# HyeonwooNoh/VQA-Transfer-ExternalData

Hardware: AMD Instinct MI355X
Metric: VQA train samples/sec (img+question) at bs512 (higher is better)
Workload: dtype f32

## Files before the change

vqa-transfer-externaldata_amd/csrc/fusion_model.hip:

```cpp
#include <stdlib.h>
#include <string.h>

#include <string>
#include <vector>

#include "gemm_args.h"
#include "gru_encoder.h"
#include "keep_launch.h"

namespace {

inline bool has_tuned_head(int mt) { return mt == VQA_MODEL_VQA_ALL2 || mt == VQA_MODEL_VQA_ALL; }
inline bool train_loss_masked(int mt) { return mt != VQA_MODEL_STANDARD; }
inline bool bf16_routed(int mt) { return mt == VQA_MODEL_VLMAP_ANSWER || mt == VQA_MODEL_STANDARD; }
inline bool feat16(const vqa_dims_t& d) { return (d.flags & VQA_FLAG_BF16_FEATURES) != 0; }

void legacy_vqa_layout(Layout& L, const vqa_dims_t& d, int64_t& gw);

Layout make_layout(const vqa_dims_t& d) {
    Layout L;
    const int64_t B = d.B, R = d.R, D = d.D, H = d.H, T = d.T, W = d.W, A = d.A;
    L.add("V_ft", B * R * D, feat16(d) ? 2 : 4);
    L.add("num_V_ft", B);
    L.add("pre_v", B * R * H);
// ... 244 lines not shown
int run_chains(const Ctx& c, int64_t B, Fn fn) {
    Chains& ch = gru_chains();
    int n = ch.n;
    while (n > 1 && B < 64 * (int64_t)n) --n;
    if (n <= 1) return fn(0, (int64_t)0, B, c.st);
    if (hipEventRecord(ch.fork, c.st) != hipSuccess) return VQA_ERR_LAUNCH;
    int rc = VQA_OK, launched = 0;
    for (int i = 1; i < n && rc == VQA_OK; ++i) {
        int64_t lo, hi;
        chain_rows(B, n, i, &lo, &hi);
        if (hipStreamWaitEvent(ch.s[i], ch.fork, 0) != hipSuccess) { rc = VQA_ERR_LAUNCH; break; }
        launched = i;
        if (ch.delay_us > 0.f) rc = vqa_stream_delay_us(ch.delay_us * (float)i, ch.s[i]);
        if (rc == VQA_OK) rc = fn(i, lo, hi - lo, ch.s[i]);
    }
    if (rc == VQA_OK) {
        int64_t lo, hi;
        chain_rows(B, n, 0, &lo, &hi);
        rc = fn(0, lo, hi - lo, c.st);
    }
    for (int i = 1; i <= launched; ++i)
        if (hipEventRecord(ch.join[i], ch.s[i]) != hipSuccess || hipStreamWaitEvent(c.st, ch.join[i], 0) != hipSuccess)
            rc = rc == VQA_OK ? VQA_ERR_LAUNCH : rc;
    return rc;
}
bool fork_side(const Ctx& c, Side& sd) {
    if (!sd.ok) return false;
    return hipEventRecord(sd.fork, c.st) == hipSuccess && hipStreamWaitEvent(sd.s, sd.fork, 0) == hipSuccess;
}
bool join_side_record(Side& sd) { return hipEventRecord(sd.join, sd.s) == hipSuccess; }


int gemm_f32(const Ctx& c, int tA, int tB, int64_t M, int64_t N, int64_t K, const float* A, int lda, const float* B,
             int ldb, float* C, int ldc, const float* bias = nullptr, const float* D = nullptr, int ldd = 0) {
    return vqa_gemm_f32_ex(tA, tB, (int)M, (int)N, (int)K, A, lda, B, ldb, C, ldc, bias, D, ldd, 0, c.gemm_ws(),
                           c.gemm_ws_floats(), c.lane ? side_max_blocks() : 0, c.st);
}
int gemm(const Ctx& c, int tA, int tB, int64_t M, int64_t N, int64_t K, const float* A, int lda, const float* B,
         int ldb, float* C, int ldc, const float* bias = nullptr, const float* D = nullptr, int ldd = 0) {
    if (c.d.flags & VQA_FLAG_BF16_GEMM)
        return vqa_gemm_bf16(tA, tB, (int)M, (int)N, (int)K, A, lda, B, ldb, C, ldc, bias, D, ldd, 0, c.gemm_ws(),
                             c.gemm_ws_floats(), c.lane ? side_max_blocks() : 0, c.st);
    return gemm_f32(c, tA, tB, M, N, K, A, lda, B, ldb, C, ldc, bias, D, ldd);
}
int gemm_x(const Ctx& c, int tA, int64_t M, int64_t N, int64_t K, const float* x, int ldx, const float* B, int ldb, float* C,
           int ldc, const float* bias = nullptr) {
    if (feat16(c.d) && x == c.f("V_ft"))
        return vqa_gemm_bf16_a16(tA, 0, (int)M, (int)N, (int)K, c.u16("V_ft"), ldx, B, ldb, C, ldc, bias, nullptr, 0, 0,
                                 c.gemm_ws(), c.gemm_ws_floats(), c.lane ? side_max_blocks() : 0, c.st);
    return gemm(c, tA, 0, M, N, K, x, ldx, B, ldb, C, ldc, bias);
}
int colsum(const Ctx& c, const float* X, int64_t M, int64_t N, int ldx, float* out) {
    return vqa_colsum(X, (int)M, (int)N, ldx, out, c.colsum_ws(), c.colsum_ws_floats(), c.st);
}
auto f32(const Ctx& c) { return [&c](auto... a) { return gemm_f32(c, a...); }; }
GruCell fw_cell(const vqa_params_t* p) { return {p->gru_wg, p->gru_bg, p->gru_wc, p->gru_bc}; }
GruCell bw_cell(const vqa_params_t* p) { return {p->gru_bw_wg, p->gru_bw_bg, p->gru_bw_wc, p->gru_bw_bc}; }

bool dims_ok(const vqa_dims_t* d) {
    if (!(d && d->B > 0 && d->R > 0 && d->D > 0 && d->H > 0 && d->T > 0 && d->W > 0 && d->A > 0 && d->Vq > 0 &&
          d->N_img > 0 && d->model_type >= VQA_MODEL_VLMAP_ANSWER && d->model_type <= VQA_MODEL_LEGACY_VQA))
        return false;
    if ((d->flags & VQA_FLAG_BF16_GEMM) && (!bf16_routed(d->model_type) || (d->flags & VQA_FLAG_FUSED_GATHER))) return false;
    if ((d->flags & VQA_FLAG_BF16_FEATURES) && !(d->flags & VQA_FLAG_BF16_GEMM)) return false;
    if (d->flags & VQA_PT_FLAG_BF16_ENCODER) return false;
    if (d->model_type == VQA_MODEL_LEGACY_VQA)
        return d->map_dim > 0 && d->La > 0 && d->H % 4 == 0 && d->D % 4 == 0 && d->map_dim % 4 == 0 && d->W % 4 == 0 && d->H <= 1024 && d->Vq > 3;
    if (d->model_type == VQA_MODEL_BI) return d->H % 8 == 0;
    if (d->model_type == VQA_MODEL_ENT)
        return d->num_marginal > 0 && d->ent_cols > 0 && d->ent_cols <= d->A && d->ent_cols <= 4096 &&
               (int64_t)d->B * d->num_marginal * (2 * (int64_t)d->H > d->ent_cols ? 2 * (int64_t)d->H : d->ent_cols) < (1ll << 30);
    return true;
}
inline int64_t pooled_dim(const vqa_dims_t& d) { return d.model_type == VQA_MODEL_ADAPT ? d.H : d.D; }

struct KeepSite {
    const uint8_t* mask;
    bool seeded;
    uint64_t seed, off;
    KeepSrc src(float keep_prob, int64_t row_len) const {
        return seeded ? KeepSrc::seeded(seed, off, row_len, keep_prob) : KeepSrc::bytes(mask, keep_prob);
    }
};
const KeepSite NO_KEEP = {nullptr, false, 0, 0};

KeepSite keep_site(const vqa_batch_t* bt, int site) {
    const bool sd = (bt->keep_seeded & site) != 0;
    switch (site) {
// ... 202 lines not shown
    return VQA_OK;
}

extern "C" int vqa_vtail_set_mode(int mode) {
    g_vtail_mode = mode < 0 ? -1 : (mode ? 1 : 0);
    return vtail_mode();
}

extern "C" int vqa_gru_h0skip_set_mode(int mode) {
    g_h0skip_mode = mode < 0 ? -1 : (mode & 3);
    return h0skip_mode();
}

namespace {

struct Step {
    const vqa_dims_t& d;
    const vqa_params_t* const P;
    const vqa_params_t* const G;
    const vqa_batch_t* const bt;
    const Layout L;
    const Ctx c;
    const int mt;
    const int64_t B, R, D, H, T, W, A;
    const int64_t Dp;
    GruTape enc[2];
    Side* sd = nullptr;
    bool forked = false;
    bool fuse_gather = false, visual_late = false;
    const float* q_ft = nullptr;
    const float* qv_in = nullptr;
    const float* lin_in = nullptr;
    bool pair = false;

    Step(const vqa_dims_t* dims, const vqa_params_t* P_, const vqa_params_t* G_, const vqa_batch_t* bt_, void* workspace,
         void* stream)
        : d(*dims), P(P_), G(G_), bt(bt_), L(make_layout(*dims)),
          c{{L, static_cast<char*>(workspace)}, *dims, static_cast<hipStream_t>(stream), 0}, mt(dims->model_type),
          B(dims->B), R(dims->R), D(dims->D), H(dims->H), T(dims->T), W(dims->W), A(dims->A),
          Dp(pooled_dim(*dims)) {
        if (mt == VQA_MODEL_LEGACY_VQA) return;
        const int64_t Hc = mt == VQA_MODEL_BI ? H / 2 : H;
        enc[0] = GruTape(c, "", "", "", T, B, Hc, W, fw_cell(P), c.st);
        if (mt == VQA_MODEL_BI) enc[1] = GruTape(c, "", "", "_bw", T, B, Hc, W, bw_cell(P), c.st);
    }
    Step(const Step&) = delete;
    Step& operator=(const Step&) = delete;

    Ctx side_ctx() const { return Ctx{{L, c.ws}, d, forked ? sd->s : c.st, forked ? 1 : 0}; }
    float* const dh = c.f("d_h0");
};

int side_record(const Step& s) { return !s.forked || join_side_record(*s.sd) ? VQA_OK : VQA_ERR_LAUNCH; }
int side_wait(const Step& s) {
    return !s.forked || hipStreamWaitEvent(s.c.st, s.sd->join, 0) == hipSuccess ? VQA_OK : VQA_ERR_LAUNCH;
}

enum GruForm { GRU_WS, GRU_LIVE, GRU_CHAINS };
enum GruDir { GRU_FWD, GRU_BWD };
GruForm gru_form(GruDir dir, int64_t T, int64_t B, int64_t H, const int32_t* live_rows) {
    const bool ws_ok = gru_ws_on() && (live_rows == nullptr || (T > 0 && live_rows[T - 1] > 0));
    if (ws_ok && (dir == GRU_FWD ? vqa_gru_ws_supported((int)T, (int)B, (int)H) : vqa_gru_ws_bwd_supported((int)T, (int)B, (int)H)) == 1)
        return GRU_WS;
    return live_rows != nullptr ? GRU_LIVE : GRU_CHAINS;
}


void fwd_visual_plan(Step& s) {
    s.sd = &side_stream();
    s.forked = fork_side(s.c, *s.sd);
    const int gm = gather_mode(&s.d);
    const bool same_kernel = gm == 2 && side_max_blocks() == 0 &&
                             vqa_gemm_gather_matches_plain((int)(s.B * s.R), (int)s.H, (int)s.D, (int)s.D, (int)s.R, s.d.N_img);
    s.fuse_gather = !(s.d.flags & VQA_FLAG_BF16_GEMM) && (gm == 1 || same_kernel) && (s.D % 32 == 0) && (s.H % 4 == 0) &&
                    vqa_aligned16(s.bt->table);
    s.visual_late = !s.forked && visual_late_enabled();
}

int fwd_visual(const Step& s) {
    const Ctx cv = s.side_ctx();
    const vqa_params_t* P = s.P;
    const vqa_batch_t* bt = s.bt;
    const int64_t B = s.B, R = s.R, D = s.D, H = s.H;
    {
        ProbeScope ps("gather", cv.st);
        if (feat16(s.d))
            TRY(vqa_gather_features_bf16(reinterpret_cast<const uint16_t*>(bt->table), bt->nbox_table, bt->image_idx,
                                         cv.u16("V_ft"), cv.i32("num_V_ft"), (int)B, (int)R, (int)D, s.d.N_img, cv.st));
        else
            TRY(vqa_gather_features(bt->table, bt->nbox_table, bt->image_idx, s.fuse_gather ? nullptr : cv.f("V_ft"),
                                    cv.i32("num_V_ft"), (int)B, (int)R, (int)D, s.d.N_img, cv.st));
    }
    if (s.fuse_gather) {
        {
            ProbeScope ps("v_linear_v.fwd_gemm", cv.st);
            TRY(vqa_gemm_f32_gather((int)(B * R), (int)H, (int)D, bt->table, (int)D, bt->image_idx, (int)R, s.d.N_img,
                                    P->v_linear_v.w, (int)H, cv.f("pre_v"), (int)H, P->v_linear_v.b, cv.f("V_ft"), (int)D,
                                    cv.st));
        }
        ProbeScope ps("v_linear_v.ln_fwd", cv.st);
        TRY(vqa_ln_relu_fwd(cv.f("pre_v"), P->v_linear_v.gamma, P->v_linear_v.beta, nullptr, 1.f, cv.f("v_linear_v"),
                            cv.f("mean_v"), cv.f("rstd_v"), (int)B, (int)R, (int)H, cv.st));
    } else {
        TRY(fc_ln_relu_fwd(cv, cv.f("V_ft"), B * R, D, H, P->v_linear_v, (int)R, "pre_v", "v_linear_v", "mean_v", "rstd_v",
                           NO_KEEP, 1.f));
    }
    if (s.mt == VQA_MODEL_ADAPT) {
        VQA_REQUIRE(P->v_adapt.w != nullptr && P->v_adapt.gamma != nullptr, VQA_ERR_ARG);
        TRY(fc_ln_relu_fwd(cv, cv.f("V_ft"), B * R, D, H, P->v_adapt, (int)R, "pre_va", "v_adapt", "mean_va", "rstd_va",
                           NO_KEEP, 1.f));
    }
    return VQA_OK;
}

int fwd_question(Step& s) {
    const Ctx& c = s.c;
    const vqa_params_t* P = s.P;
    const vqa_batch_t* bt = s.bt;
    const int64_t B = s.B, H = s.H, T = s.T, W = s.W;
    if (s.mt == VQA_MODEL_BI) {
        TRY(bi_question_fwd(c, P, bt, s.enc));
        s.q_ft = c.f("q_L_ft");
        s.qv_in = c.f("pooled_q_v");
        return VQA_OK;
    }
    const GruTape& e = s.enc[0];
    {
        ProbeScope ps("embed.fwd", c.st);
        TRY(vqa_embed_fwd_ld(P->embed, bt->q_intseq, e.x_tm, (int)B, (int)T, (int)W, s.d.Vq, e.ldx(), c.st));
    }
    {
        ProbeScope ps("gru.xp_gemm", c.st);
        if (xcat_enabled()) {
            TRY(e.pack_wx());
            TRY(e.project(f32(c)));
        } else {
            TRY(gemm_f32(c, 0, 0, T * B, 2 * H, W, e.x_tm, e.ldx(), P->gru_wg, (int)(2 * H), e.xp, (int)(3 * H), P->gru_bg));
            TRY(gemm_f32(c, 0, 0, T * B, H, W, e.x_tm, e.ldx(), P->gru_wc, (int)H, e.xp + 2 * H, (int)(3 * H), P->gru_bc));
        }
    }
    TRY(e.clear_h0());
    const float *Wg_h = e.Wg_h(), *Wc_h = e.Wc_h();
    {
        ProbeScope ps("gru.fwd", c.st);
        switch (gru_form(GRU_FWD, T, B, H, bt->live_rows)) {
            case GRU_WS:
                TRY(vqa_gru_seq_fwd_ws_ex(e.xp, Wg_h, Wc_h, bt->q_intseq_len, e.hs, e.gru_r, e.gru_u, e.gru_c, e.gru_rh, (int)T, (int)B,
                                          (int)H, h0skip_mode() & 1, c.find_f("gru_ws"), c.st));
                break;
            case GRU_LIVE:
                TRY(vqa_gru_seq_fwd_live(e.xp, Wg_h, Wc_h, bt->q_intseq_len, bt->live_rows, e.hs, e.gru_r, e.gru_u, e.gru_c, e.gru_rh,
                                         (int)T, (int)B, (int)H, c.st));
                break;
            case GRU_CHAINS:
                TRY(run_chains(c, B, [&](int, int64_t row0, int64_t rows, hipStream_t st) {
                    return vqa_gru_seq_fwd_rows(e.xp, Wg_h, Wc_h, bt->q_intseq_len, e.hs, e.gru_r, e.gru_u, e.gru_c, e.gru_rh, (int)T,
                                                (int)B, (int)H, (int)row0, (int)rows, st);
                }));
                break;
        }
    }
    s.q_ft = e.h_final();
    s.qv_in = s.q_ft;
    return VQA_OK;
}

int fwd_question_code(Step& s) {
    const Ctx& c = s.c;
    const vqa_params_t* P = s.P;
    const int64_t B = s.B, H = s.H;
    const float* h = s.q_ft;
    s.lin_in = h;
    if (s.mt == VQA_MODEL_ANSWER2) {
        VQA_REQUIRE(P->q_L_ft2.w != nullptr && P->q_L_ft2.gamma != nullptr, VQA_ERR_ARG);
// ... 410 lines not shown
                          "rstd_qv", NO_KEEP, 1.f, "d_pre_qv", s.dh, true);
}

int bwd_bptt(const Step& s, float* embed_slice_sq) {
    const Ctx& c = s.c;
    const vqa_params_t* P = s.P;
    const vqa_batch_t* bt = s.bt;
    const int64_t B = s.B, H = s.H, T = s.T, W = s.W;
    const GruTape& e = s.enc[0];
    float* dh = s.dh;
    const float *Wg_h = e.Wg_h(), *Wc_h = e.Wc_h();
    {
        ProbeScope ps("gru.bwd", c.st);
        switch (gru_form(GRU_BWD, T, B, H, bt->live_rows)) {
            case GRU_WS:
                TRY(vqa_gru_seq_bwd_ws_ex(dh, nullptr, Wg_h, Wc_h, bt->q_intseq_len, e.hs, e.gru_r, e.gru_u, e.gru_c, e.dxp, (int)T, (int)B,
                                          (int)H, h0skip_mode() & 1, c.find_f("gru_ws"), c.st));
                break;
            case GRU_LIVE:
                TRY(vqa_gru_seq_bwd_live(dh, Wg_h, Wc_h, bt->q_intseq_len, bt->live_rows, e.hs, e.gru_r, e.gru_u, e.gru_c, e.dxp,
                                         c.f("d_h1"), (int)T, (int)B, (int)H, c.st));
                break;
            case GRU_CHAINS: {
                float* dh1 = c.f("d_h1");
                TRY(run_chains(c, B, [&](int, int64_t row0, int64_t rows, hipStream_t st) {
                    return vqa_gru_seq_bwd_rows(dh, Wg_h, Wc_h, bt->q_intseq_len, e.hs, e.gru_r, e.gru_u, e.gru_c, e.dxp, dh1, (int)T,
                                                (int)B, (int)H, (int)row0, (int)rows, st);
                }));
                break;
            }
        }
    }
    float* dx = c.f("dx_embed");
    {
        ProbeScope ps("gru.dx_gemm", c.st);
        if (xcat_enabled()) {
            if (repack_enabled()) TRY(e.pack_wx());
            TRY(e.dx(f32(c), dx));
        } else {
            TRY(gemm_f32(c, 0, 1, T * B, W, 2 * H, e.dxp, (int)(3 * H), P->gru_wg, (int)(2 * H), dx, (int)W));
            TRY(gemm_f32(c, 0, 1, T * B, W, H, e.dxp + 2 * H, (int)(3 * H), P->gru_wc, (int)H, dx, (int)W, nullptr, dx, (int)W));
        }
    }
    ProbeScope ps_embed("embed.bwd", c.st);
    if (s.G->embed != nullptr)
        TRY(vqa_embed_bwd_len_det(dx, bt->q_intseq, bt->q_intseq_len, s.G->embed, (int)B, (int)T, (int)W, s.d.Vq,
                                  (s.d.flags & VQA_FLAG_DETERMINISTIC) ? 1 : 0, c.st));
    if (embed_slice_sq != nullptr)
        TRY(vqa_sumsq(dx, T * B * W, nullptr, embed_slice_sq, c.f("sumsq_ws"), c.count("sumsq_ws"), c.st));
    return VQA_OK;
}

int bwd_gru_weights(const Ctx& c, const GruTape& e, const GruCell& g, int phases, bool packed, int t0) {
    const int64_t TB = e.T * e.B, H = e.H, W = e.W;
    const int ld3 = (int)(3 * H);
    if (g.wg == nullptr) return VQA_OK;
    if (phases & 4) {
        {
            ProbeScope ps("gru.dwx_gemm", c.st);
            if (packed) {
                TRY(e.dwx(f32(c)));
                TRY(e.unpack_dwx(g));
            } else {
                TRY(gemm_f32(c, 1, 0, W, 2 * H, TB, e.x_tm, e.ldx(), e.dxp, ld3, g.wg, (int)(2 * H)));
                TRY(colsum(c, e.dxp, TB, 2 * H, ld3, g.bg));
            }
        }
        ProbeScope ps("gru.dwh_gemm", c.st);
        TRY(e.dwh(f32(c), g, false, t0));
    }
    if (phases & 8) {
        if (!packed) {
            ProbeScope ps("gru.dwx_gemm", c.st);
            TRY(gemm_f32(c, 1, 0, W, H, TB, e.x_tm, e.ldx(), e.dxp + 2 * H, ld3, g.wc, (int)H));
            TRY(colsum(c, e.dxp + 2 * H, TB, H, ld3, g.bc));
        }
        ProbeScope ps("gru.dwh_gemm", c.st);
        TRY(e.dwh(f32(c), g, true, t0));
    }
    return VQA_OK;
}

}

extern "C" int vqa_fusion_backward_phases(const vqa_dims_t* dims, const vqa_params_t* P, const vqa_params_t* G,
                                          const vqa_batch_t* bt, void* workspace, int64_t workspace_bytes,
                                          float* embed_slice_sq, int phases, void* stream) {
    VQA_REQUIRE(dims_ok(dims) && P && G && bt && workspace, VQA_ERR_ARG);
    VQA_REQUIRE(keep_sites_ok(bt), VQA_ERR_ARG);
    Step s(dims, P, G, bt, workspace, stream);
    VQA_REQUIRE(workspace_bytes >= s.L.total, VQA_ERR_WORKSPACE);
    ProbeScope ps_all("backward", s.c.st);
    if (s.mt == VQA_MODEL_LEGACY_VQA) return (phases & 1) ? legacy_vqa_backward(s.c, P, G, bt, embed_slice_sq) : VQA_OK;
    s.pair = ln_pair_ok(s.d, P);

    if (phases & 1) {
        TRY(bwd_head(s));
        TRY(bwd_joint(s));
        if (s.mt == VQA_MODEL_ENT) TRY(bwd_entropy(s));
        TRY(bwd_linear_l(s));
        TRY(bwd_question_code(s));
        TRY(bwd_attention(s));
        TRY(bwd_q_linear_v(s));
        TRY(side_wait(s));
    }
    if (s.mt == VQA_MODEL_BI) {
        if (phases & 2) TRY(bi_question_bwd_bptt(s.c, G, bt, s.enc, s.dh, embed_slice_sq));
        TRY(bwd_gru_weights(s.c, s.enc[0], fw_cell(G), phases, true, 0));
        return bwd_gru_weights(s.c, s.enc[1], bw_cell(G), phases, true, 0);
    }
    if (phases & 2) TRY(bwd_bptt(s, embed_slice_sq));
    return (phases & 12) ? bwd_gru_weights(s.c, s.enc[0], fw_cell(G), phases, xcat_enabled(), (h0skip_mode() >> 1) & 1) : VQA_OK;
}

extern "C" int vqa_hot_version(void) { return VQA_HOT_ABI_VERSION; }

extern "C" const char* vqa_hot_error_string(int code) {
    switch (code) {
        case VQA_OK: return "ok";
        case VQA_ERR_ARG: return "bad argument (size or null pointer)";
        case VQA_ERR_ALIGN: return "pointer / leading dimension not aligned";
        case VQA_ERR_LAUNCH: return "kernel launch failed";
        case VQA_ERR_UNSUPPORTED: return "unsupported configuration";
        case VQA_ERR_WORKSPACE: return "workspace too small";
        default: return "unknown error";
    }
}
```

vqa-transfer-externaldata_amd/csrc/gemm_args.h:

```cpp
#pragma once
#include <hip/hip_runtime.h>
#include <stdint.h>

struct GemmArgs {
    int M, N, K;
    const float* A; int lda;
    const float* B; int ldb;
    float* C; int ldc;
    const float* bias;
    const float* D; int ldd;
    int k_per_split;
    int64_t slab_stride;
    int vecA, vecB;
    int tiles_m, tiles_n, nsplit;
    int m_fastest;
    unsigned a_bytes, b_bytes;
    const float* scale;
    int relu;
    int Hi, Wi, Ci, Ho, Wo, cstride, pad_t, pad_l, kw;
    int conv_taps;
    int vec_epi;
    const int64_t* g_idx; int g_R; int64_t g_N; float* g_out; int g_ldo;
};

enum { EPI_PLAIN = 0, EPI_GATES = 1, EPI_CAND = 2, EPI_BWD_RH = 3, EPI_BWD_DH = 4 };
struct EpiArgs {
    int H, t, ldo;
    const int32_t* len;
    const float* h_prev;
    const float* i0;
    const float* i1;
    float* o0;
    float* o1;
    float* o2;
};

GemmArgs vqa_gemm_make_args(int M, int N, int K, const float* A, int lda, const float* B, int ldb, float* C, int ldc,
                            const float* bias, const float* D, int ldd);
bool vqa_gemm_gather_matches_plain(int M, int N, int K, int lda, int R, int64_t n_samples_in_table);
int vqa_gru_step_launch(int epi, int cfg, const GemmArgs& a, const EpiArgs& ep, hipStream_t st);
int vqa_gru_step_launch_bf16(int epi, const GemmArgs& a, const EpiArgs& ep, hipStream_t st);
bool vqa_gru_cfg_known(int cfg);
int vqa_gru_rs_launch(int epi, const GemmArgs& a, const EpiArgs& ep, hipStream_t st);
```

vqa-transfer-externaldata_amd/csrc/gemm_f32.hip:

```cpp

#include "vqa_common.h"
#include "gemm_args.h"
#include "gemm_tiles.h"
#include <cstdio>
#include <cstdlib>

#ifndef VQA_GEMM_STAGGER
#define VQA_GEMM_STAGGER 1
#endif

typedef float f32x16 __attribute__((ext_vector_type(16)));
typedef unsigned int u32x4 __attribute__((ext_vector_type(4)));

#if defined(VQA_DBG_STAMPS)
__device__ unsigned long long* g_dbg_stamps = nullptr;
#define DBG_STAMP(i) do { if (threadIdx.x == 0) dbg_t[i] = __builtin_amdgcn_s_memrealtime(); } while (0)
#else
#define DBG_STAMP(i) do {} while (0)
#endif

namespace {


__device__ __forceinline__ int xcd_remap(int lin, int total) {
// ... 948 lines not shown
}
extern "C" int vqa_gemm_shortk_set_mode(int mode) {
    g_shortk_mode = mode < 0 ? -1 : (mode & 3);
    return VQA_OK;
}

extern "C" int vqa_gemm_f32(int transA, int transB, int M, int N, int K, const float* A, int lda, const float* B,
                            int ldb, float* C, int ldc, const float* bias, const float* D, int ldd, int split_k,
                            float* workspace, int64_t workspace_floats, void* stream) {
    return vqa_gemm_f32_ex(transA, transB, M, N, K, A, lda, B, ldb, C, ldc, bias, D, ldd, split_k, workspace,
                           workspace_floats, g_max_blocks, stream);
}

#if defined(VQA_DBG_STAMPS)
extern "C" int vqa_gemm_dbg_stamps(void* buf) {
    unsigned long long* b = static_cast<unsigned long long*>(buf);
    return hipMemcpyToSymbol(HIP_SYMBOL(g_dbg_stamps), &b, sizeof(b)) == hipSuccess ? VQA_OK : VQA_ERR_LAUNCH;
}
#endif

extern "C" int vqa_gemm_set_order(int order) {
    g_force_order = (order == 0 || order == 1) ? order : -1;
    return VQA_OK;
}

extern "C" int vqa_gemm_set_max_blocks(int n) {
    g_max_blocks = n > 0 ? n : 0;
    return VQA_OK;
}

extern "C" int vqa_gemm_f32_ex(int transA, int transB, int M, int N, int K, const float* A, int lda, const float* B,
                               int ldb, float* C, int ldc, const float* bias, const float* D, int ldd, int split_k,
                               float* workspace, int64_t workspace_floats, int max_blocks, void* stream) {
    VQA_REQUIRE(M >= 0 && N >= 0 && K >= 0, VQA_ERR_ARG);
    if (M == 0 || N == 0) return VQA_OK;
    VQA_REQUIRE(A && B && C, VQA_ERR_ARG);
    VQA_REQUIRE(!(transA == 1 && transB == 1), VQA_ERR_UNSUPPORTED);
    VQA_REQUIRE(lda >= (transA ? M : K) && ldb >= (transB ? K : N) && ldc >= N, VQA_ERR_ARG);
    VQA_REQUIRE(D == nullptr || ldd >= N, VQA_ERR_ARG);
    hipStream_t st = static_cast<hipStream_t>(stream);

    if (bf16x3_mode() && !transB && D == nullptr && max_blocks == 0 && g_force_cfg < 0 && vqa_gemm_bf16x3_supported(M, N, K) &&
        (int64_t)M * N * K >= (1ll << 32) && lda % 4 == 0 && ldb % 4 == 0 && vqa_aligned16(A) && vqa_aligned16(B)) {
        const int tiles = (M / 128) * (N / 128);
        int sp = 1;
        while (tiles * sp < 256 && K / (sp * 2) >= 512 && sp < 16) sp *= 2;
        while (sp > 1 && (workspace == nullptr || workspace_floats < (int64_t)sp * M * N || ldc % 4 != 0 || !vqa_aligned16(C))) sp /= 2;
        return vqa_gemm_bf16x3(transA, M, N, K, A, lda, B, ldb, C, ldc, bias, sp, workspace, workspace_floats, stream);
    }
    if (!transA && !transB && split_k <= 1 && max_blocks == 0 && g_force_cfg < 0 && (shortk_mode() & 1) &&
        M >= 1024 && K <= 304 && vqa_gemm_shortk_supported(M, N, K, lda, ldb, ldc) && !(K > 256 && D != nullptr) && vqa_aligned16(A) &&
        vqa_aligned16(B))
        return vqa_gemm_shortk_nn(M, N, K, A, lda, B, ldb, C, ldc, bias, nullptr, D, ldd, 0, stream);

    int cfg, split = split_k;
    choose(transA, transB, M, N, K, cfg, split);
    if (split > 1 && ((N % 4) != 0 || workspace == nullptr)) split = 1;

    GemmArgs a = vqa_gemm_make_args(M, N, K, A, lda, B, ldb, C, ldc, bias, D, ldd);
    if (split > 1) {
        VQA_REQUIRE(workspace_floats >= (int64_t)split * M * N, VQA_ERR_WORKSPACE);
        int kps = (int)cdiv(cdiv(K, split), 64) * 64;
        a.k_per_split = kps;
        split = (int)cdiv(K, kps);
    }
    if (split > 1) {
        a.C = workspace; a.ldc = N; a.slab_stride = (int64_t)M * N;
        int rc = launch_by_id(cfg, transA, transB, a, split, st, max_blocks);
        if (rc != VQA_OK) return rc;
        const int64_t n4 = (int64_t)M * N / 4;
        const int grid = (int)std::min<int64_t>(cdiv(n4, 256), 2048);
        hipLaunchKernelGGL(splitk_reduce_kernel, dim3(grid), dim3(256), 0, st, workspace, C, M, N, ldc, split);
        VQA_CHECK_LAUNCH();
        return VQA_OK;
    }
    a.k_per_split = (int)cdiv(std::max(K, 1), 64) * 64;
    return launch_by_id(cfg, transA, transB, a, 1, st, max_blocks);
}

extern "C" int vqa_gemm_f32_gather(int M, int N, int K, const float* table, int lda, const int64_t* idx, int R,
                                   int64_t n_samples_in_table, const float* B, int ldb, float* C, int ldc,
                                   const float* bias, float* gathered_out, int ldg, void* stream) {
    VQA_REQUIRE(M >= 0 && N >= 0 && K > 0 && R > 0 && n_samples_in_table > 0, VQA_ERR_ARG);
    if (M == 0 || N == 0) return VQA_OK;
    VQA_REQUIRE(table && idx && B && C, VQA_ERR_ARG);
    VQA_REQUIRE(lda >= K && ldb >= N && ldc >= N && (gathered_out == nullptr || ldg >= K), VQA_ERR_ARG);
    VQA_REQUIRE(K % 32 == 0 && N % 4 == 0, VQA_ERR_UNSUPPORTED);
    VQA_REQUIRE(lda % 4 == 0 && vqa_aligned16(table) && ldb % 4 == 0 && vqa_aligned16(B) &&
                    (gathered_out == nullptr || (ldg % 4 == 0 && vqa_aligned16(gathered_out))),
                VQA_ERR_ALIGN);
    GemmArgs a = vqa_gemm_make_args(M, N, K, table, lda, B, ldb, C, ldc, bias, nullptr, 0);
    const int64_t bb = ((int64_t)(K - 1) * ldb + N) * 4;
    VQA_REQUIRE(bb < 0xFFFFFF00ll, VQA_ERR_UNSUPPORTED);
    const int64_t ab = ((n_samples_in_table * R - 1) * (int64_t)lda + K) * 4;
    const bool by_offset = !g_gather_ptr && ab < 0xFFFFFF00ll;
    a.a_bytes = by_offset ? (unsigned)ab : 0;
    a.b_bytes = (unsigned)bb;
    VQA_REQUIRE(gathered_out == nullptr || ((int64_t)(M - 1) * ldg + K) * 4 < 0xFFFFFF00ll, VQA_ERR_UNSUPPORTED);
    a.g_idx = idx; a.g_R = R; a.g_N = n_samples_in_table; a.g_out = gathered_out; a.g_ldo = ldg;
    a.k_per_split = (int)cdiv(K, 64) * 64;
    const EpiArgs ep{};
    hipStream_t st = static_cast<hipStream_t>(stream);
// ... 86 lines not shown
```

vqa-transfer-externaldata_amd/csrc/gru_encoder.h:

```cpp
#pragma once
#include "step_workspace.h"
#include "vqa_common.h"

struct GruCell { float *wg, *bg, *wc, *bc; };

struct GruTape {
    float *x_tm, *xp, *wx_cat, *bx_cat, *dwx_cat, *hs, *gru_r, *gru_u, *gru_c, *gru_rh, *dxp;
    int64_t T, B, H, W;
    GruCell p;
    hipStream_t st;
    GruTape() = default;
    GruTape(const Workspace& w, const std::string& tape, const std::string& scratch, const std::string& suffix, int64_t T_,
            int64_t B_, int64_t H_, int64_t W_, const GruCell& p_, hipStream_t st_)
        : T(T_), B(B_), H(H_), W(W_), p(p_), st(st_) {
        auto in = [&](const char* n) { return w.f(tape + n + suffix); };
        auto scr = [&](const char* n) { return w.f(scratch + n + suffix); };
        x_tm = in("x_tm"); xp = in("xp"); hs = in("hs");
        gru_r = in("gru_r"); gru_u = in("gru_u"); gru_c = in("gru_c"); gru_rh = in("gru_rh");
        wx_cat = scr("wx_cat"); bx_cat = scr("bx_cat"); dwx_cat = scr("dwx_cat"); dxp = scr("dxp");
    }
    int ldx() const { return (int)x_stride(W); }
    const float* Wg_h() const { return p.wg + W * 2 * H; }
    const float* Wc_h() const { return p.wc + W * H; }
    float* h_final() const { return hs + T * B * H; }

    int pack_wx() const { return vqa_gru_pack_wx(p.wg, p.wc, p.bg, p.bc, wx_cat, bx_cat, (int)W, (int)H, st); }
    template <class Gemm>
    int project(Gemm&& gemm) const {
        return gemm(0, 0, T * B, 3 * H, W, x_tm, ldx(), wx_cat, (int)(3 * H), xp, (int)(3 * H), bx_cat);
    }
    int clear_h0() const { return hipMemsetAsync(hs, 0, (size_t)(B * H) * 4, st) == hipSuccess ? VQA_OK : VQA_ERR_LAUNCH; }
    template <class Gemm>
    int dx(Gemm&& gemm, float* dx_out) const {
        return gemm(0, 1, T * B, W, 3 * H, dxp, (int)(3 * H), wx_cat, (int)(3 * H), dx_out, (int)W, nullptr);
    }
    template <class Gemm>
    int dwx(Gemm&& gemm) const {
        return gemm(1, 0, x_stride(W), 3 * H, T * B, x_tm, ldx(), dxp, (int)(3 * H), dwx_cat, (int)(3 * H), nullptr);
    }
    int unpack_dwx(const GruCell& g) const { return vqa_gru_unpack_dwx_bias(dwx_cat, g.wg, g.wc, g.bg, g.bc, (int)W, (int)H, st); }
    template <class Gemm>
    int dwh(Gemm&& gemm, const GruCell& g, bool cand, int t0) const {
        const int64_t N = cand ? H : 2 * H, row0 = t0 * B;
        float* dW = cand ? g.wc + W * H : g.wg + W * 2 * H;
        if (t0 >= T) return hipMemsetAsync(dW, 0, (size_t)(H * N) * 4, st) == hipSuccess ? VQA_OK : VQA_ERR_LAUNCH;
        return gemm(1, 0, H, N, (T - t0) * B, (cand ? gru_rh : hs) + row0 * H, (int)H, dxp + row0 * 3 * H + (cand ? 2 * H : 0),
                    (int)(3 * H), dW, (int)N, nullptr);
    }
};
```

vqa-transfer-externaldata_amd/csrc/rowops.hip:

```cpp
#include "vqa_common.h"

namespace {

inline int64_t cdiv(int64_t a, int64_t b) { return (a + b - 1) / b; }
inline int grid_for(int64_t work_items, int cap = 4096) {
    return (int)std::max<int64_t>(1, std::min<int64_t>(cdiv(work_items, 256), cap));
}

__global__ __launch_bounds__(256) void gather_features_kernel(const float* __restrict__ table,
                                                              const int32_t* __restrict__ nbox_table,
                                                              const int64_t* __restrict__ idx, float* __restrict__ V,
                                                              int32_t* __restrict__ nb, int B, int64_t row_floats,
                                                              int64_t N) {
    const int b = blockIdx.x;
    int64_t src = idx[b];
    if (src < 0) src = 0;
    if (src >= N) src = N - 1;
    if (blockIdx.y == 0 && threadIdx.x == 0 && nb != nullptr) nb[b] = nbox_table[src];
    const float* s = table + src * row_floats;
    float* d = V + (int64_t)b * row_floats;
    const int64_t n4 = row_floats / 4;
    for (int64_t i = blockIdx.y * 256 + threadIdx.x; i < n4; i += (int64_t)gridDim.y * 256)
        reinterpret_cast<float4*>(d)[i] = reinterpret_cast<const float4*>(s)[i];
    if (blockIdx.y == 0)
        for (int64_t i = n4 * 4 + threadIdx.x; i < row_floats; i += 256) d[i] = s[i];
}

template <typename VT>
__global__ __launch_bounds__(256) void gather_features_bf16_kernel(const uint16_t* __restrict__ table,
                                                                   const int32_t* __restrict__ nbox_table,
                                                                   const int64_t* __restrict__ idx, uint16_t* __restrict__ V,
                                                                   int32_t* __restrict__ nb, int B, int64_t row_elems,
// ... 344 lines not shown
}

__global__ __launch_bounds__(256) void pack_wx_kernel(const float* __restrict__ wg, const float* __restrict__ wc,
                                                      const float* __restrict__ bg, const float* __restrict__ bc,
                                                      float* __restrict__ wx, float* __restrict__ bx, int W, int H) {
    const int H3 = 3 * H;
    const int64_t n = (int64_t)W * H3;
    for (int64_t i = (int64_t)blockIdx.x * 256 + threadIdx.x; i < n + H3; i += (int64_t)gridDim.x * 256) {
        if (i < n) {
            const int r = (int)(i / H3), col = (int)(i - (int64_t)r * H3);
            wx[i] = col < 2 * H ? wg[(int64_t)r * 2 * H + col] : wc[(int64_t)r * H + (col - 2 * H)];
        } else {
            const int col = (int)(i - n);
            bx[col] = col < 2 * H ? bg[col] : bc[col - 2 * H];
        }
    }
}
__global__ __launch_bounds__(256) void unpack_dwx_kernel(const float* __restrict__ dwx, float* __restrict__ gwg,
                                                         float* __restrict__ gwc, float* __restrict__ gbg,
                                                         float* __restrict__ gbc, int W, int H) {
    const int H3 = 3 * H;
    const int64_t n = (int64_t)(W + (gbg != nullptr ? 1 : 0)) * H3;
    for (int64_t i = (int64_t)blockIdx.x * 256 + threadIdx.x; i < n; i += (int64_t)gridDim.x * 256) {
        const int r = (int)(i / H3), col = (int)(i - (int64_t)r * H3);
        if (r < W) {
            if (col < 2 * H) gwg[(int64_t)r * 2 * H + col] = dwx[i];
            else gwc[(int64_t)r * H + (col - 2 * H)] = dwx[i];
        } else {
            if (col < 2 * H) gbg[col] = dwx[i];
            else gbc[col - 2 * H] = dwx[i];
        }
    }
}
}

extern "C" int vqa_gru_pack_wx(const float* wg, const float* wc, const float* bg, const float* bc, float* wx, float* bx, int W,
                               int H, void* stream) {
    VQA_REQUIRE(wg && wc && bg && bc && wx && bx && W > 0 && H > 0, VQA_ERR_ARG);
    const int64_t n = (int64_t)W * 3 * H + 3 * H;
    hipLaunchKernelGGL(pack_wx_kernel, dim3((unsigned)std::min<int64_t>((n + 255) / 256, 2048)), dim3(256), 0,
                       (hipStream_t)stream, wg, wc, bg, bc, wx, bx, W, H);
    VQA_CHECK_LAUNCH();
    return VQA_OK;
}

extern "C" int vqa_gru_unpack_dwx(const float* dwx, float* gwg, float* gwc, int W, int H, void* stream) {
    return vqa_gru_unpack_dwx_bias(dwx, gwg, gwc, nullptr, nullptr, W, H, stream);
}

extern "C" int vqa_gru_unpack_dwx_bias(const float* dwx, float* gwg, float* gwc, float* gbg, float* gbc, int W, int H,
                                       void* stream) {
    VQA_REQUIRE(dwx && gwg && gwc && W > 0 && H > 0 && (gbg == nullptr) == (gbc == nullptr), VQA_ERR_ARG);
    const int64_t n = (int64_t)(W + 1) * 3 * H;
    hipLaunchKernelGGL(unpack_dwx_kernel, dim3((unsigned)std::min<int64_t>((n + 255) / 256, 2048)), dim3(256), 0,
                       (hipStream_t)stream, dwx, gwg, gwc, gbg, gbc, W, H);
    VQA_CHECK_LAUNCH();
    return VQA_OK;
}

extern "C" int vqa_gather_features(const float* table, const int32_t* nbox_table, const int64_t* idx, float* V,
                                   int32_t* nb, int B, int R, int D, int64_t N, void* stream) {
    VQA_REQUIRE(table && idx && (V || nb) && B >= 0 && R > 0 && D > 0 && N > 0, VQA_ERR_ARG);
    VQA_REQUIRE(nb == nullptr || nbox_table != nullptr, VQA_ERR_ARG);
    VQA_REQUIRE(vqa_aligned16(table) && vqa_aligned16(V) && ((int64_t)R * D) % 4 == 0, VQA_ERR_ALIGN);
    if (B == 0) return VQA_OK;
    const int64_t row = V != nullptr ? (int64_t)R * D : 0;
// ... 327 lines not shown
```

Measured before the change: 166,500.

## Fuse encoder prologue and fold split-K reductions into embed/dwx finish kernels

Replaces the separate embedding lookup, wx packing, h0 clearing and nbox gather with one multi-role prologue kernel. In the backward pass, split-K GEMMs for dx and dwx can now hand back unreduced slabs, and a single finish kernel sums them and scatters into the embedding gradient or the unpacked weight gradients. The aim is to cut kernel launches and extra passes over memory on the encoder path. It adds more code paths gated by an env flag, and the dx path uses atomics so it is skipped when deterministic mode is on.

```diff
diff --git a/vqa-transfer-externaldata_amd/csrc/encoder_launches.h b/vqa-transfer-externaldata_amd/csrc/encoder_launches.h
--- /dev/null
+++ b/vqa-transfer-externaldata_amd/csrc/encoder_launches.h
@@ -0,0 +1,13 @@
+#pragma once
+#include <hip/hip_runtime.h>
+#include <stdint.h>
+
+int vqa_encoder_prologue(const float* E, const int32_t* q, float* x_tm, int B, int T, int W, int Vq, int ldx, const float* wg,
+                         const float* wc, const float* bg, const float* bc, float* wx, float* bx, int H, float* h0,
+                         const int32_t* nbox_table, const int64_t* idx, int32_t* nb, int64_t N_img, hipStream_t st);
+
+int vqa_encoder_dx_finish(const float* slabs, int split, float* dx, const int32_t* q, const int32_t* len, float* dE, int B,
+                          int T, int W, int Vq, hipStream_t st);
+
+int vqa_encoder_dwx_finish(const float* slabs, int split, float* dwx, int rows, float* gwg, float* gwc, float* gbg, float* gbc,
+                           int W, int H, hipStream_t st);
diff --git a/vqa-transfer-externaldata_amd/csrc/fusion_model.hip b/vqa-transfer-externaldata_amd/csrc/fusion_model.hip
--- a/vqa-transfer-externaldata_amd/csrc/fusion_model.hip
+++ b/vqa-transfer-externaldata_amd/csrc/fusion_model.hip
@@ -300,9 +300,10 @@
 
 
 int gemm_f32(const Ctx& c, int tA, int tB, int64_t M, int64_t N, int64_t K, const float* A, int lda, const float* B,
-             int ldb, float* C, int ldc, const float* bias = nullptr, const float* D = nullptr, int ldd = 0) {
-    return vqa_gemm_f32_ex(tA, tB, (int)M, (int)N, (int)K, A, lda, B, ldb, C, ldc, bias, D, ldd, 0, c.gemm_ws(),
-                           c.gemm_ws_floats(), c.lane ? side_max_blocks() : 0, c.st);
+             int ldb, float* C, int ldc, const float* bias = nullptr, const float* D = nullptr, int ldd = 0,
+             int* slabs_left = nullptr) {
+    return vqa_gemm_f32_slabs(tA, tB, (int)M, (int)N, (int)K, A, lda, B, ldb, C, ldc, bias, D, ldd, 0, c.gemm_ws(),
+                              c.gemm_ws_floats(), c.lane ? side_max_blocks() : 0, slabs_left, c.st);
 }
 int gemm(const Ctx& c, int tA, int tB, int64_t M, int64_t N, int64_t K, const float* A, int lda, const float* B,
          int ldb, float* C, int ldc, const float* bias = nullptr, const float* D = nullptr, int ldd = 0) {
@@ -322,6 +323,10 @@
     return vqa_colsum(X, (int)M, (int)N, ldx, out, c.colsum_ws(), c.colsum_ws_floats(), c.st);
 }
 auto f32(const Ctx& c) { return [&c](auto... a) { return gemm_f32(c, a...); }; }
+auto f32_slabs(const Ctx& c, int* split) {
+    return [&c, split](int tA, int tB, int64_t M, int64_t N, int64_t K, const float* A, int lda, const float* B, int ldb, float* C,
+                       int ldc, const float* bias) { return gemm_f32(c, tA, tB, M, N, K, A, lda, B, ldb, C, ldc, bias, nullptr, 0, split); };
+}
 GruCell fw_cell(const vqa_params_t* p) { return {p->gru_wg, p->gru_bg, p->gru_wc, p->gru_bc}; }
 GruCell bw_cell(const vqa_params_t* p) { return {p->gru_bw_wg, p->gru_bw_bg, p->gru_bw_wc, p->gru_bw_bc}; }
 
@@ -590,6 +595,8 @@
     const float* qv_in = nullptr;
     const float* lin_in = nullptr;
     bool pair = false;
+    const bool enc_launches = env_on("VQA_HOT_ENC_LAUNCHES", true);
+    bool enc_nbox = false;
 
     Step(const vqa_dims_t* dims, const vqa_params_t* P_, const vqa_params_t* G_, const vqa_batch_t* bt_, void* workspace,
          void* stream)
@@ -624,6 +631,10 @@
 }
 
 
+bool enc_prologue_on(const Step& s) {
+    return s.enc_launches && s.mt != VQA_MODEL_BI && s.mt != VQA_MODEL_LEGACY_VQA && xcat_enabled();
+}
+
 void fwd_visual_plan(Step& s) {
     s.sd = &side_stream();
     s.forked = fork_side(s.c, *s.sd);
@@ -633,6 +644,7 @@
     s.fuse_gather = !(s.d.flags & VQA_FLAG_BF16_GEMM) && (gm == 1 || same_kernel) && (s.D % 32 == 0) && (s.H % 4 == 0) &&
                     vqa_aligned16(s.bt->table);
     s.visual_late = !s.forked && visual_late_enabled();
+    s.enc_nbox = enc_prologue_on(s) && s.fuse_gather && !s.forked && !feat16(s.d);
 }
 
 int fwd_visual(const Step& s) {
@@ -640,7 +652,7 @@
     const vqa_params_t* P = s.P;
     const vqa_batch_t* bt = s.bt;
     const int64_t B = s.B, R = s.R, D = s.D, H = s.H;
-    {
+    if (!s.enc_nbox) {
         ProbeScope ps("gather", cv.st);
         if (feat16(s.d))
             TRY(vqa_gather_features_bf16(reinterpret_cast<const uint16_t*>(bt->table), bt->nbox_table, bt->image_idx,
@@ -683,21 +695,26 @@
         return VQA_OK;
     }
     const GruTape& e = s.enc[0];
+    const bool folded = enc_prologue_on(s);
     {
         ProbeScope ps("embed.fwd", c.st);
-        TRY(vqa_embed_fwd_ld(P->embed, bt->q_intseq, e.x_tm, (int)B, (int)T, (int)W, s.d.Vq, e.ldx(), c.st));
+        if (folded)
+            TRY(e.prologue(P->embed, bt->q_intseq, s.d.Vq, bt->nbox_table, bt->image_idx, s.enc_nbox ? c.i32("num_V_ft") : nullptr,
+                           s.d.N_img));
+        else
+            TRY(vqa_embed_fwd_ld(P->embed, bt->q_intseq, e.x_tm, (int)B, (int)T, (int)W, s.d.Vq, e.ldx(), c.st));
     }
     {
         ProbeScope ps("gru.xp_gemm", c.st);
         if (xcat_enabled()) {
-            TRY(e.pack_wx());
+            if (!folded) TRY(e.pack_wx());
             TRY(e.project(f32(c)));
         } else {
             TRY(gemm_f32(c, 0, 0, T * B, 2 * H, W, e.x_tm, e.ldx(), P->gru_wg, (int)(2 * H), e.xp, (int)(3 * H), P->gru_bg));
             TRY(gemm_f32(c, 0, 0, T * B, H, W, e.x_tm, e.ldx(), P->gru_wc, (int)H, e.xp + 2 * H, (int)(3 * H), P->gru_bc));
         }
     }
-    TRY(e.clear_h0());
+    if (!folded) TRY(e.clear_h0());
     const float *Wg_h = e.Wg_h(), *Wc_h = e.Wc_h();
     {
         ProbeScope ps("gru.fwd", c.st);
@@ -1174,18 +1191,23 @@
         }
     }
     float* dx = c.f("dx_embed");
+    const bool folded = s.enc_launches && xcat_enabled() && s.G->embed != nullptr && !(s.d.flags & VQA_FLAG_DETERMINISTIC);
+    int dx_split = 1;
     {
         ProbeScope ps("gru.dx_gemm", c.st);
         if (xcat_enabled()) {
             if (repack_enabled()) TRY(e.pack_wx());
-            TRY(e.dx(f32(c), dx));
+            if (folded) TRY(e.dx(f32_slabs(c, &dx_split), dx));
+            else TRY(e.dx(f32(c), dx));
         } else {
             TRY(gemm_f32(c, 0, 1, T * B, W, 2 * H, e.dxp, (int)(3 * H), P->gru_wg, (int)(2 * H), dx, (int)W));
             TRY(gemm_f32(c, 0, 1, T * B, W, H, e.dxp + 2 * H, (int)(3 * H), P->gru_wc, (int)H, dx, (int)W, nullptr, dx, (int)W));
         }
     }
     ProbeScope ps_embed("embed.bwd", c.st);
-    if (s.G->embed != nullptr)
+    if (folded)
+        TRY(e.finish_dx(c.gemm_ws(), dx_split, dx, bt->q_intseq, bt->q_intseq_len, s.G->embed, s.d.Vq));
+    else if (s.G->embed != nullptr)
         TRY(vqa_embed_bwd_len_det(dx, bt->q_intseq, bt->q_intseq_len, s.G->embed, (int)B, (int)T, (int)W, s.d.Vq,
                                   (s.d.flags & VQA_FLAG_DETERMINISTIC) ? 1 : 0, c.st));
     if (embed_slice_sq != nullptr)
@@ -1193,14 +1215,18 @@
     return VQA_OK;
 }
 
-int bwd_gru_weights(const Ctx& c, const GruTape& e, const GruCell& g, int phases, bool packed, int t0) {
+int bwd_gru_weights(const Ctx& c, const GruTape& e, const GruCell& g, int phases, bool packed, int t0, bool folded) {
     const int64_t TB = e.T * e.B, H = e.H, W = e.W;
     const int ld3 = (int)(3 * H);
     if (g.wg == nullptr) return VQA_OK;
     if (phases & 4) {
         {
             ProbeScope ps("gru.dwx_gemm", c.st);
-            if (packed) {
+            if (packed && folded) {
+                int split = 1;
+                TRY(e.dwx(f32_slabs(c, &split)));
+                TRY(e.finish_dwx(c.gemm_ws(), split, g));
+            } else if (packed) {
                 TRY(e.dwx(f32(c)));
                 TRY(e.unpack_dwx(g));
             } else {
@@ -1248,11 +1274,12 @@
     }
     if (s.mt == VQA_MODEL_BI) {
         if (phases & 2) TRY(bi_question_bwd_bptt(s.c, G, bt, s.enc, s.dh, embed_slice_sq));
-        TRY(bwd_gru_weights(s.c, s.enc[0], fw_cell(G), phases, true, 0));
-        return bwd_gru_weights(s.c, s.enc[1], bw_cell(G), phases, true, 0);
+        TRY(bwd_gru_weights(s.c, s.enc[0], fw_cell(G), phases, true, 0, s.enc_launches));
+        return bwd_gru_weights(s.c, s.enc[1], bw_cell(G), phases, true, 0, s.enc_launches);
     }
     if (phases & 2) TRY(bwd_bptt(s, embed_slice_sq));
-    return (phases & 12) ? bwd_gru_weights(s.c, s.enc[0], fw_cell(G), phases, xcat_enabled(), (h0skip_mode() >> 1) & 1) : VQA_OK;
+    return (phases & 12) ? bwd_gru_weights(s.c, s.enc[0], fw_cell(G), phases, xcat_enabled(), (h0skip_mode() >> 1) & 1, s.enc_launches)
+                         : VQA_OK;
 }
 
 extern "C" int vqa_hot_version(void) { return VQA_HOT_ABI_VERSION; }
diff --git a/vqa-transfer-externaldata_amd/csrc/gemm_args.h b/vqa-transfer-externaldata_amd/csrc/gemm_args.h
--- a/vqa-transfer-externaldata_amd/csrc/gemm_args.h
+++ b/vqa-transfer-externaldata_amd/csrc/gemm_args.h
@@ -37,6 +37,9 @@
 
 GemmArgs vqa_gemm_make_args(int M, int N, int K, const float* A, int lda, const float* B, int ldb, float* C, int ldc,
                             const float* bias, const float* D, int ldd);
+int vqa_gemm_f32_slabs(int transA, int transB, int M, int N, int K, const float* A, int lda, const float* B, int ldb,
+                       float* C, int ldc, const float* bias, const float* D, int ldd, int split_k, float* workspace,
+                       int64_t workspace_floats, int max_blocks, int* slabs_left, hipStream_t stream);
 bool vqa_gemm_gather_matches_plain(int M, int N, int K, int lda, int R, int64_t n_samples_in_table);
 int vqa_gru_step_launch(int epi, int cfg, const GemmArgs& a, const EpiArgs& ep, hipStream_t st);
 int vqa_gru_step_launch_bf16(int epi, const GemmArgs& a, const EpiArgs& ep, hipStream_t st);
diff --git a/vqa-transfer-externaldata_amd/csrc/gemm_f32.hip b/vqa-transfer-externaldata_amd/csrc/gemm_f32.hip
--- a/vqa-transfer-externaldata_amd/csrc/gemm_f32.hip
+++ b/vqa-transfer-externaldata_amd/csrc/gemm_f32.hip
@@ -1004,6 +1004,14 @@
 extern "C" int vqa_gemm_f32_ex(int transA, int transB, int M, int N, int K, const float* A, int lda, const float* B,
                                int ldb, float* C, int ldc, const float* bias, const float* D, int ldd, int split_k,
                                float* workspace, int64_t workspace_floats, int max_blocks, void* stream) {
+    return vqa_gemm_f32_slabs(transA, transB, M, N, K, A, lda, B, ldb, C, ldc, bias, D, ldd, split_k, workspace,
+                              workspace_floats, max_blocks, nullptr, static_cast<hipStream_t>(stream));
+}
+
+int vqa_gemm_f32_slabs(int transA, int transB, int M, int N, int K, const float* A, int lda, const float* B, int ldb,
+                       float* C, int ldc, const float* bias, const float* D, int ldd, int split_k, float* workspace,
+                       int64_t workspace_floats, int max_blocks, int* slabs_left, hipStream_t stream) {
+    if (slabs_left != nullptr) *slabs_left = 1;
     VQA_REQUIRE(M >= 0 && N >= 0 && K >= 0, VQA_ERR_ARG);
     if (M == 0 || N == 0) return VQA_OK;
     VQA_REQUIRE(A && B && C, VQA_ERR_ARG);
@@ -1040,6 +1048,10 @@
         a.C = workspace; a.ldc = N; a.slab_stride = (int64_t)M * N;
         int rc = launch_by_id(cfg, transA, transB, a, split, st, max_blocks);
         if (rc != VQA_OK) return rc;
+        if (slabs_left != nullptr && ldc == N) {
+            *slabs_left = split;
+            return VQA_OK;
+        }
         const int64_t n4 = (int64_t)M * N / 4;
         const int grid = (int)std::min<int64_t>(cdiv(n4, 256), 2048);
         hipLaunchKernelGGL(splitk_reduce_kernel, dim3(grid), dim3(256), 0, st, workspace, C, M, N, ldc, split);
diff --git a/vqa-transfer-externaldata_amd/csrc/gru_encoder.h b/vqa-transfer-externaldata_amd/csrc/gru_encoder.h
--- a/vqa-transfer-externaldata_amd/csrc/gru_encoder.h
+++ b/vqa-transfer-externaldata_amd/csrc/gru_encoder.h
@@ -1,4 +1,5 @@
 #pragma once
+#include "encoder_launches.h"
 #include "step_workspace.h"
 #include "vqa_common.h"
 
@@ -39,6 +40,17 @@
         return gemm(1, 0, x_stride(W), 3 * H, T * B, x_tm, ldx(), dxp, (int)(3 * H), dwx_cat, (int)(3 * H), nullptr);
     }
     int unpack_dwx(const GruCell& g) const { return vqa_gru_unpack_dwx_bias(dwx_cat, g.wg, g.wc, g.bg, g.bc, (int)W, (int)H, st); }
+    int prologue(const float* embed, const int32_t* q, int Vq, const int32_t* nbox_table, const int64_t* image_idx, int32_t* nb,
+                 int64_t N_img) const {
+        return vqa_encoder_prologue(embed, q, x_tm, (int)B, (int)T, (int)W, Vq, ldx(), p.wg, p.wc, p.bg, p.bc, wx_cat, bx_cat,
+                                    (int)H, hs, nbox_table, image_idx, nb, N_img, st);
+    }
+    int finish_dx(const float* slabs, int split, float* dx_out, const int32_t* q, const int32_t* len, float* d_embed, int Vq) const {
+        return vqa_encoder_dx_finish(slabs, split, dx_out, q, len, d_embed, (int)B, (int)T, (int)W, Vq, st);
+    }
+    int finish_dwx(const float* slabs, int split, const GruCell& g) const {
+        return vqa_encoder_dwx_finish(slabs, split, dwx_cat, (int)x_stride(W), g.wg, g.wc, g.bg, g.bc, (int)W, (int)H, st);
+    }
     template <class Gemm>
     int dwh(Gemm&& gemm, const GruCell& g, bool cand, int t0) const {
         const int64_t N = cand ? H : 2 * H, row0 = t0 * B;
diff --git a/vqa-transfer-externaldata_amd/csrc/rowops.hip b/vqa-transfer-externaldata_amd/csrc/rowops.hip
--- a/vqa-transfer-externaldata_amd/csrc/rowops.hip
+++ b/vqa-transfer-externaldata_amd/csrc/rowops.hip
@@ -1,3 +1,4 @@
+#include "encoder_launches.h"
 #include "vqa_common.h"
 
 namespace {
@@ -408,6 +409,230 @@
         }
     }
 }
+
+template <bool VEC>
+__global__ __launch_bounds__(256) void encoder_prologue_kernel(const float* __restrict__ E, const int32_t* __restrict__ q,
+                                                               float* __restrict__ x, int B, int T, int W, int Vq, int ldx,
+                                                               const float* __restrict__ wg, const float* __restrict__ wc,
+                                                               const float* __restrict__ bg, const float* __restrict__ bc,
+                                                               float* __restrict__ wx, float* __restrict__ bx, int H,
+                                                               float* __restrict__ h0, const int32_t* __restrict__ nbox_table,
+                                                               const int64_t* __restrict__ idx, int32_t* __restrict__ nb,
+                                                               int64_t N, int ne, int np, int nz) {
+    int blk = blockIdx.x;
+    if (blk < ne) {
+        const int tok = blk * 4 + (threadIdx.x >> 6);
+        if (tok >= B * T) return;
+        const int t = tok / B, b = tok % B;
+        int id = q[b * T + t];
+        id = min(max(id, 0), Vq - 1);
+        const float* s = E + (int64_t)id * W;
+        float* d = x + (int64_t)tok * ldx;
+        if (VEC) {
+            const int w4 = W / 4;
+            for (int i = threadIdx.x & 63; i < ldx / 4; i += 64)
+                reinterpret_cast<float4*>(d)[i] = i < w4 ? reinterpret_cast<const float4*>(s)[i]
+                                                         : make_float4(i == w4 ? 1.f : 0.f, 0.f, 0.f, 0.f);
+        } else {
+            for (int i = threadIdx.x & 63; i < ldx; i += 64) d[i] = i < W ? s[i] : (i == W ? 1.f : 0.f);
+        }
+        return;
+    }
+    blk -= ne;
+    const int H3 = 3 * H;
+    if (blk < np) {
+        const int64_t n = (int64_t)W * H3;
+        if (VEC) {
+            for (int64_t i = (int64_t)blk * 256 + threadIdx.x; i < (n + H3) / 4; i += (int64_t)np * 256) {
+                const int64_t e = i * 4;
+                const float* s;
+                if (e < n) {
+                    const int r = (int)(e / H3), col = (int)(e - (int64_t)r * H3);
+                    s = col < 2 * H ? wg + (int64_t)r * 2 * H + col : wc + (int64_t)r * H + (col - 2 * H);
+                } else {
+                    const int col = (int)(e - n);
+                    s = col < 2 * H ? bg + col : bc + (col - 2 * H);
+                }
+                float* d = e < n ? wx + e : bx + (e - n);
+                *reinterpret_cast<float4*>(d) = *reinterpret_cast<const float4*>(s);
+            }
+        } else {
+            for (int64_t i = (int64_t)blk * 256 + threadIdx.x; i < n + H3; i += (int64_t)np * 256) {
+                if (i < n) {
+                    const int r = (int)(i / H3), col = (int)(i - (int64_t)r * H3);
+                    wx[i] = col < 2 * H ? wg[(int64_t)r * 2 * H + col] : wc[(int64_t)r * H + (col - 2 * H)];
+                } else {
+                    const int col = (int)(i - n);
+                    bx[col] = col < 2 * H ? bg[col] : bc[col - 2 * H];
+                }
+            }
+        }
+        return;
+    }
+    blk -= np;
+    if (blk < nz) {
+        const int64_t n = (int64_t)B * H;
+        if (VEC) {
+            for (int64_t i = (int64_t)blk * 256 + threadIdx.x; i < n / 4; i += (int64_t)nz * 256)
+                reinterpret_cast<float4*>(h0)[i] = make_float4(0.f, 0.f, 0.f, 0.f);
+        } else {
+            for (int64_t i = (int64_t)blk * 256 + threadIdx.x; i < n; i += (int64_t)nz * 256) h0[i] = 0.f;
+        }
+        return;
+    }
+    blk -= nz;
+    const int b = blk * 256 + threadIdx.x;
+    if (b < B) {
+        int64_t src = idx[b];
+        if (src < 0) src = 0;
+        if (src >= N) src = N - 1;
+        nb[b] = nbox_table[src];
+    }
+}
+
+__device__ __forceinline__ float4 slab_sum4(const float* __restrict__ slabs, int64_t i, int64_t MN, int S) {
+    float4 a = reinterpret_cast<const float4*>(slabs)[i];
+    for (int z = 1; z < S; ++z) {
+        const float4 b = reinterpret_cast<const float4*>(slabs + (int64_t)z * MN)[i];
+        a.x += b.x; a.y += b.y; a.z += b.z; a.w += b.w;
+    }
+    return a;
+}
+__device__ __forceinline__ float slab_sum1(const float* __restrict__ slabs, int64_t i, int64_t MN, int S) {
+    float a = slabs[i];
+    for (int z = 1; z < S; ++z) a += slabs[(int64_t)z * MN + i];
+    return a;
+}
+
+template <bool VEC>
+__global__ __launch_bounds__(256) void encoder_dx_finish_kernel(const float* slabs, int S, float* dx,
+                                                                const int32_t* __restrict__ q, const int32_t* __restrict__ len,
+                                                                float* __restrict__ dE, int B, int T, int W, int Vq) {
+    const int64_t MN = (int64_t)T * B * W;
+    if (VEC) {
+        __shared__ __attribute__((aligned(16))) float stage[1024];
+        const unsigned n = (unsigned)MN, chunks = (n + 1023u) / 1024u;
+        for (unsigned c = blockIdx.x; c < chunks; c += gridDim.x) {
+            const unsigned e0 = c * 1024u, i = e0 / 4u + threadIdx.x;
+            if (i < n / 4u) {
+                const float4 a = slab_sum4(slabs, i, MN, S);
+                if (S > 1) reinterpret_cast<float4*>(dx)[i] = a;
+                reinterpret_cast<float4*>(stage)[threadIdx.x] = a;
+            }
+            __syncthreads();
+#pragma unroll
+            for (int k = 0; k < 4; ++k) {
+                const unsigned j = k * 256u + threadIdx.x, e = e0 + j;
+                if (e >= n) break;
+                const unsigned tok = e / (unsigned)W, col = e - tok * (unsigned)W;
+                const int t = (int)(tok / (unsigned)B), b = (int)(tok % (unsigned)B);
+                if (len != nullptr && t >= len[b]) continue;
+                int id = q[b * T + t];
+                id = min(max(id, 0), Vq - 1);
+                atomicAdd(dE + (int64_t)id * W + col, stage[j]);
+            }
+            __syncthreads();
+        }
+        return;
+    }
+    for (int64_t i = (int64_t)blockIdx.x * 256 + threadIdx.x; i < MN; i += (int64_t)gridDim.x * 256) {
+        const int tok = (int)(i / W), col = (int)(i - (int64_t)tok * W);
+        const int t = tok / B, b = tok % B;
+        const bool live = len == nullptr || t < len[b];
+        if (S == 1 && !live) continue;
+        const float v = slab_sum1(slabs, i, MN, S);
+        if (S > 1) dx[i] = v;
+        if (!live) continue;
+        int id = q[b * T + t];
+        id = min(max(id, 0), Vq - 1);
+        atomicAdd(dE + (int64_t)id * W + col, v);
+    }
+}
+
+template <bool VEC>
+__global__ __launch_bounds__(256) void encoder_dwx_finish_kernel(const float* slabs, int S, float* dwx, int rows,
+                                                                 float* __restrict__ gwg, float* __restrict__ gwc,
+                                                                 float* __restrict__ gbg, float* __restrict__ gbc, int W, int H,
+                                                                 bool dvec) {
+    const int H3 = 3 * H;
+    const int64_t MN = (int64_t)rows * H3;
+    constexpr int V = VEC ? 4 : 1;
+    for (int64_t i = (int64_t)blockIdx.x * 256 + threadIdx.x; i < MN / V; i += (int64_t)gridDim.x * 256) {
+        const int64_t e = i * V;
+        const int r = (int)(e / H3), col = (int)(e - (int64_t)r * H3);
+        float* d = nullptr;
+        if (r < W) d = col < 2 * H ? gwg + (int64_t)r * 2 * H + col : gwc + (int64_t)r * H + (col - 2 * H);
+        else if (r == W && gbg != nullptr) d = col < 2 * H ? gbg + col : gbc + (col - 2 * H);
+        if (S == 1 && d == nullptr) continue;
+        float v[4];
+        if (VEC) {
+            const float4 a = slab_sum4(slabs, i, MN, S);
+            if (S > 1) reinterpret_cast<float4*>(dwx)[i] = a;
+            v[0] = a.x; v[1] = a.y; v[2] = a.z; v[3] = a.w;
+        } else {
+            v[0] = slab_sum1(slabs, i, MN, S);
+            if (S > 1) dwx[i] = v[0];
+        }
+        if (d == nullptr) continue;
+        if (VEC && dvec) {
+            *reinterpret_cast<float4*>(d) = make_float4(v[0], v[1], v[2], v[3]);
+        } else {
+#pragma unroll
+            for (int k = 0; k < V; ++k) d[k] = v[k];
+        }
+    }
+}
+}
+
+int vqa_encoder_prologue(const float* E, const int32_t* q, float* x_tm, int B, int T, int W, int Vq, int ldx, const float* wg,
+                         const float* wc, const float* bg, const float* bc, float* wx, float* bx, int H, float* h0,
+                         const int32_t* nbox_table, const int64_t* idx, int32_t* nb, int64_t N_img, hipStream_t st) {
+    VQA_REQUIRE(E && q && x_tm && B > 0 && T > 0 && W > 0 && Vq > 0 && ldx >= W, VQA_ERR_ARG);
+    VQA_REQUIRE(wg && wc && bg && bc && wx && bx && H > 0 && h0, VQA_ERR_ARG);
+    VQA_REQUIRE(nb == nullptr || (nbox_table != nullptr && idx != nullptr && N_img > 0), VQA_ERR_ARG);
+    const int64_t n_pack = (int64_t)W * 3 * H + 3 * H;
+    const int ne = (B * T + 3) / 4;
+    const int np = (int)std::min<int64_t>((n_pack + 255) / 256, 2048);
+    const int nz = (int)std::min<int64_t>(cdiv((int64_t)B * H, 256 * 4), 2048);
+    const int nn = nb != nullptr ? (B + 255) / 256 : 0;
+    const bool vec = W % 4 == 0 && ldx % 4 == 0 && H % 4 == 0 && vqa_aligned16(E) && vqa_aligned16(x_tm) && vqa_aligned16(wg) &&
+                     vqa_aligned16(wc) && vqa_aligned16(bg) && vqa_aligned16(bc) && vqa_aligned16(wx) && vqa_aligned16(bx) &&
+                     vqa_aligned16(h0);
+    auto kern = vec ? encoder_prologue_kernel<true> : encoder_prologue_kernel<false>;
+    hipLaunchKernelGGL(kern, dim3((unsigned)(ne + np + nz + nn)), dim3(256), 0, st, E, q, x_tm, B, T, W, Vq, ldx, wg, wc, bg, bc,
+                       wx, bx, H, h0, nbox_table, idx, nb, N_img, ne, np, nz);
+    VQA_CHECK_LAUNCH();
+    return VQA_OK;
+}
+
+int vqa_encoder_dx_finish(const float* slabs, int split, float* dx, const int32_t* q, const int32_t* len, float* dE, int B,
+                          int T, int W, int Vq, hipStream_t st) {
+    VQA_REQUIRE(dx && q && dE && B >= 0 && T >= 0 && W > 0 && Vq > 0 && split >= 1 && (split == 1 || slabs != nullptr), VQA_ERR_ARG);
+    if (B * T == 0) return VQA_OK;
+    const float* src = split > 1 ? slabs : dx;
+    const int64_t MN = (int64_t)T * B * W;
+    const bool vec = W % 4 == 0 && MN < (1ll << 31) && vqa_aligned16(src) && vqa_aligned16(dx);
+    const int grid = (int)std::max<int64_t>(1, std::min<int64_t>(cdiv(MN, vec ? 1024 : 256), 2048));
+    auto kern = vec ? encoder_dx_finish_kernel<true> : encoder_dx_finish_kernel<false>;
+    hipLaunchKernelGGL(kern, dim3(grid), dim3(256), 0, st, src, split, dx, q, len, dE, B, T, W, Vq);
+    VQA_CHECK_LAUNCH();
+    return VQA_OK;
+}
+
+int vqa_encoder_dwx_finish(const float* slabs, int split, float* dwx, int rows, float* gwg, float* gwc, float* gbg, float* gbc,
+                           int W, int H, hipStream_t st) {
+    VQA_REQUIRE(dwx && gwg && gwc && W > 0 && H > 0 && rows >= W + (gbg != nullptr ? 1 : 0) && (gbg == nullptr) == (gbc == nullptr) &&
+                    split >= 1 && (split == 1 || slabs != nullptr),
+                VQA_ERR_ARG);
+    const float* src = split > 1 ? slabs : dwx;
+    const bool vec = H % 4 == 0 && vqa_aligned16(src) && vqa_aligned16(dwx);
+    const int64_t n = (int64_t)rows * 3 * H / (vec ? 4 : 1);
+    const int grid = (int)std::max<int64_t>(1, std::min<int64_t>(cdiv(n, 256), 2048));
+    auto kern = vec ? encoder_dwx_finish_kernel<true> : encoder_dwx_finish_kernel<false>;
+    const bool dvec = vqa_aligned16(gwg) && vqa_aligned16(gwc) && vqa_aligned16(gbg) && vqa_aligned16(gbc);
+    hipLaunchKernelGGL(kern, dim3(grid), dim3(256), 0, st, src, split, dwx, rows, gwg, gwc, gbg, gbc, W, H, dvec);
+    VQA_CHECK_LAUNCH();
+    return VQA_OK;
 }
 
 extern "C" int vqa_gru_pack_wx(const float* wg, const float* wc, const float* bg, const float* bc, float* wx, float* bx, int W,
```

Result: no change. 167,100 (median of 6 runs) (+0.4%).
